# deflect-ca/banjax

Measured on AMD Instinct MI355X. Metric: log lines/sec matched+rate-limited (node) at 1k rules; HBM GB/s vs peak, higher is better.
Workload: dtype u8

## Files before the change

### banjax_amd/csrc/engine.hip

```cpp
#include <hip/hip_runtime.h>
#include <hipcub/hipcub.hpp>

#include <algorithm>
#include <array>
#include <atomic>
#include <cstdio>
#include <cstdlib>
#include <cstring>
#include <map>
#include <tuple>
#include <memory>
#include <mutex>
#include <stdexcept>
#include <string>
#include <unordered_map>
#include <thread>
#include <vector>

#include "../../include/banjax_gpu.h"
#include "bjx_common.h"
#include "engine_types.h"
#include "regex_compiler.h"
#include "bans.h"

// ... 379 lines not shown
  hid = host_lookup(B, p + host_off, host_len);
  exempt = B.any_allow && check_is_allowed(B, hid, p + ip_off, ip_len);
  L.ip_len[j] = ip_len;
  L.rest_off[j] = rest_off;
  L.host_id[j] = hid;
  {
    uint4 k16;
    uint64_t h;
    ip_key_hash(p + ip_off, ip_len, k16, h);
    if (ip_len > 15) L.ip_hash[j] = h;
    L.ip16[j] = k16;
  }
  if (!SLOW) {
    if (parse_float_fast(p, sp1, &f) != 0) {
      L.flags[j] = kLineSlowTs;
      unsigned long long k = atomicAdd(slow_count, 1ull);
      slow_list[k] = (uint32_t)j;
      return;
    }
  } else if (parse_float_fast(p, sp1, &f) != 0) {
    Decimal dec;
    if (go_parse_float(p, sp1, &f, &dec) != 0) { L.flags[j] = kLineError; return; }
  }
  const int64_t ts = ns_from_seconds(f);
  L.ts[j] = ts;
  if (go_sub(now_ns, ts) > 10000000000LL) fl = kLineOld;
  else if (exempt) fl = kLineExempt;
  L.flags[j] = fl;
  if (fl) return;

  const uint8_t *rest = p + rest_off;
  const uint32_t rest_len = n - rest_off;
  uint64_t word = 0;
  uint32_t pos = 0, wi = 0, nres = 0, nev = 0;
  uint32_t s_begin = 0, s_end = 0;
  if (hid >= 0) { s_begin = B.site_off[hid]; s_end = B.site_off[hid + 1]; }
  const uint32_t napp = (s_end - s_begin) + B.n_global;
  if (SLOW && napp > 128 && B.any_prefilter) {
    decide_wide(B, p, s, n, rest_off, hid, j, L, WL);
    return;
  }
  for (uint32_t k = 0; k < napp; ++k) {
    const uint32_t r = k < s_end - s_begin ? B.site_rules[s_begin + k] : B.global_rules[k - (s_end - s_begin)];
    if (B.any_wide && (B.rules[r].flags & kRuleNfaWide)) {
      const unsigned long long q = atomicAdd(WL.count, 1ull);
      if (q < WL.cap) { WL.line[q] = (uint32_t)j; WL.rule[q] = r; WL.pos[q] = pos; }
    } else if (rule_match(B, r, rest, rest_len)) {
      word |= 1ull << (pos & 63);
      ++nres;
      nev += is_skip(B, r, hid) ? 0u : 1u;
    }
    ++pos;
    if ((pos & 63) == 0) { L.mword(j, wi++) = word; word = 0; }
  }
  if (pos & 63) L.mword(j, wi) = word;
  L.counts[j] = ((uint64_t)nres << 32) | nev;
}

__global__ void k_no_line_pass(unsigned long long *slow_count, unsigned long long n) {
  if (threadIdx.x == 0) *slow_count = n;
}

template <bool SLOW>
__global__ __launch_bounds__(kBlock) void k_parse_match(Bind B, const uint8_t *__restrict__ buf,
                                                        const uint64_t *__restrict__ nl, uint64_t n_lines,
                                                        const uint32_t *__restrict__ list, int64_t now_ns, Lines L,
                                                        uint32_t *slow_list, unsigned long long *slow_count, WideList WL) {
  const uint64_t t = (uint64_t)blockIdx.x * blockDim.x + threadIdx.x;
  if (t >= n_lines) return;
  const uint64_t j = SLOW && list ? list[t] : t;
  const uint64_t s = j ? nl[j - 1] + 1 : 0;
  const uint32_t n = (uint32_t)(nl[j] - s);
  parse_and_match<SLOW>(B, buf + s, s, n, j, now_ns, L, slow_list, slow_count, WL);
}


constexpr uint32_t kWT = 4096;
constexpr uint32_t kHalo = 512;
constexpr uint32_t kLineCap = 128;
constexpr uint32_t kHitSlots = 4;
constexpr int kScanWaves = 16;
constexpr uint32_t kTileLds = kWT + kHalo + 16;
constexpr uint32_t kWaveJobs = 64;
constexpr uint32_t kCandList = 128;
constexpr uint32_t kBanChunks = 8;
constexpr uint64_t kBanChunkMin = 64ull << 20;
constexpr uint32_t kLongList = 64;
constexpr uint32_t kWaveLds = kTileLds + kLineCap * (2 + 2) + kCandList * 4 + kLineCap * 4 + kLongList * 8 + 16;
constexpr uint32_t kNone = 0xFFFFFFFFu;
constexpr uint32_t kScanLdsMax = 160 * 1024;
constexpr uint32_t kLinesImgMax = 16 * 1024;
constexpr uint32_t kLinesHostLdsMax = 6 * 1024;
constexpr uint32_t kLinesTabLdsMax = 10 * 1024;
constexpr uint32_t kLinesBlocksPerCu = 3;
constexpr uint32_t kSpanBytes = 12 * 1024;

__device__ __forceinline__ uint32_t space_mask16(const uint4 v) {
  const uint32_t wv[4] = {v.x, v.y, v.z, v.w};
  uint32_t m16 = 0;
#pragma unroll
  for (int k = 0; k < 4; ++k) {
    const uint32_t x = wv[k] ^ 0x20202020u;
    const uint32_t hb = ~(((x & 0x7F7F7F7Fu) + 0x7F7F7F7Fu) | x) & 0x80808080u;
    m16 |= (((hb >> 7) & 1u) | ((hb >> 14) & 2u) | ((hb >> 21) & 4u) | ((hb >> 28) & 8u)) << (4 * k);
  }
  return m16;
}

__device__ __forceinline__ bool digits4(uint32_t x) {
  return (x & 0xF0F0F0F0u) == 0x30303030u && (((x & 0x0F0F0F0Fu) + 0x06060606u) & 0xF0F0F0F0u) == 0u;
}
__device__ __forceinline__ uint32_t value4(uint32_t x) {
  x -= 0x30303030u;
  x = x * 10u + (x >> 8);
  return (x & 0xFFu) * 100u + ((x >> 16) & 0xFFu);
}
__device__ __forceinline__ int parse_ts_msec(const uint8_t *p, uint32_t n, double *out) {
  if (n != 14) return 1;
  const uint32_t w0 = ld4(p), w1 = ld4(p + 4), w2 = ld4(p + 8), w3 = ld4(p + 12);
  if (!digits4(w0) || !digits4(w1) || (w2 & 0x00FF0000u) != 0x002E0000u || !digits4((w2 & 0xFF00FFFFu) | 0x00300000u) ||
      !digits4((w3 & 0xFFFFu) | 0x30300000u))
    return 1;
  const uint32_t d8 = w2 & 0xFFu, d9 = (w2 >> 8) & 0xFFu, d11 = w2 >> 24, d12 = w3 & 0xFFu, d13 = (w3 >> 8) & 0xFFu;
  const uint64_t ip = (uint64_t)value4(w0) * 1000000ull + value4(w1) * 100u + (d8 - 48u) * 10u + (d9 - 48u);
  const uint64_t m = ip * 1000ull + (d11 - 48u) * 100u + (d12 - 48u) * 10u + (d13 - 48u);
  *out = (double)m / 1000.0;
  return 0;
}

__device__ __forceinline__ uint32_t find_spaces(const uint8_t *p, uint32_t n, uint32_t &sp0, uint32_t &sp1,
                                                uint32_t &sp2, uint32_t &sp3) {
  const uint32_t skip = (uint32_t)(reinterpret_cast<uintptr_t>(p) & 15);
  const uint4 *base = reinterpret_cast<const uint4 *>(p - skip);
  uint32_t ns = 0, c0 = 0;
  if (n + skip >= 64) {
    const uint4 v0 = base[0], v1 = base[1], v2 = base[2], v3 = base[3];
    uint64_t m = (uint64_t)space_mask16(v0) | ((uint64_t)space_mask16(v1) << 16) | ((uint64_t)space_mask16(v2) << 32) |
                 ((uint64_t)space_mask16(v3) << 48);
    m &= ~((1ull << skip) - 1ull);
#pragma unroll
    for (int k = 0; k < 4; ++k) {
      const uint32_t pos = (uint32_t)__ffsll((unsigned long long)m) - 1 - skip;
      const bool has = m != 0;
      m &= m - 1;
      if (k == 0) sp0 = has ? pos : sp0;
      if (k == 1) sp1 = has ? pos : sp1;
      if (k == 2) sp2 = has ? pos : sp2;
      if (k == 3) sp3 = has ? pos : sp3;
      ns += has ? 1u : 0u;
    }
    c0 = 4;
  }
  for (uint32_t c = c0; c * 16 < n + skip && ns < 4; ++c) {
    const uint4 v = base[c];
    uint32_t m16 = 0;
    const uint32_t wv[4] = {v.x, v.y, v.z, v.w};
#pragma unroll
    for (int k = 0; k < 4; ++k) {
      const uint32_t x = wv[k] ^ 0x20202020u;
      const uint32_t hb = ~(((x & 0x7F7F7F7Fu) + 0x7F7F7F7Fu) | x) & 0x80808080u;
      m16 |= (((hb >> 7) & 1u) | ((hb >> 14) & 2u) | ((hb >> 21) & 4u) | ((hb >> 28) & 8u)) << (4 * k);
    }
    const int32_t lo = (int32_t)skip - (int32_t)(c * 16), hi = lo + (int32_t)n;
    if (lo > 0) m16 &= ~((1u << lo) - 1u);
    if (hi < 16) m16 &= hi > 0 ? (1u << hi) - 1u : 0u;
    while (m16 && ns < 4) {
// ... 742 lines not shown
    const uint32_t lit = (uint32_t)(lits >> (16 * c)) & 0xFFFFu;
    if (lit != (a.y & 0xFFFFu) && lit != (a.y >> 16) && lit != (a.z & 0xFFFFu) && lit != (a.z >> 16)) continue;
    const uint32_t hp = (uint32_t)(lpos >> (16 * c)) & 0xFFFFu;
    if (hp == 0xFFFFu) {
      dfa_rule<EMIT>(B, T, r, pos, false, rest, rest_len, m0, m1, j, S);
      return;
    }
    const int32_t fs = side_c ? (int32_t)hp - (int32_t)host_len - (int32_t)la : (int32_t)hp;
    if (!tmpl_at(LT, a.w, rest, rest_len, host_rel, host_len, fs)) continue;
    if (eq) set_pos(m0, m1, pos);
    else dfa_rule<EMIT>(B, T, r, pos, false, rest, rest_len, m0, m1, j, S);
    return;
  }
}

template <bool EMIT>
__device__ __forceinline__ void decide_plan_lds(const Bind &B, const Tabs &T, const LdsTabs &LT, const uint8_t *rest,
                                                uint32_t rest_len, uint32_t host_rel, uint32_t host_len, int32_t hid,
                                                const HostRules &H, uint64_t lits, uint64_t lpos, uint32_t nlit, bool ovf,
                                                const OvfInfo &ov, uint64_t j, const Lines &L, const JobSink &S,
                                                LinesProf *P = nullptr) {
  const uint32_t nsite = H.s_end - H.s_begin;
  uint64_t m0 = H.a0, m1 = H.a1;
  if (P) { __builtin_amdgcn_s_waitcnt(0); P->mark(7); }
  if (hid >= 0) {
    const uint2 hi = LT.hinfo[hid];
    const uint32_t f = (uint32_t)__ffsll((unsigned long long)__ballot(1)) - 1;
    const uint32_t c0 = __builtin_amdgcn_readlane(hi.x, f);
    if (__ballot(hi.x != c0) == 0) {
      typedef const __attribute__((address_space(4))) uint32_t ConstU32;
      ConstU32 *cg = (ConstU32 *)(uintptr_t)(B.hl + B.lt_cls);
      const uint32_t cb = c0 & 0xFFFFu, ce = cb + (c0 >> 16);
      for (uint32_t i = cb; i < ce; ++i) {
        ConstU32 *q = cg + 8 * i;
        plan_rule_lds<EMIT>(B, T, LT, make_uint4(q[0], q[1], q[2], q[3]), make_uint4(q[4], q[5], q[6], q[7]), hi.y, rest, rest_len,
                            host_rel, host_len, lits, lpos, nlit, ovf, ov, m0, m1, j, S);
      }
    } else {
      const uint32_t cb = hi.x & 0xFFFFu, ce = cb + (hi.x >> 16);
      for (uint32_t i = cb; i < ce; ++i)
        plan_rule_lds<EMIT>(B, T, LT, LT.cls[2 * i], LT.cls[2 * i + 1], hi.y, rest, rest_len, host_rel, host_len, lits, lpos,
                            nlit, ovf, ov, m0, m1, j, S);
    }
  }
  if (P) { __builtin_amdgcn_s_waitcnt(0); P->mark(8); }
  for (uint32_t i = 0; i < B.n_plan_glob; ++i)
    plan_rule<EMIT>(B, T, B.plan_glob[2 * i], B.plan_glob[2 * i + 1], nsite, rest, rest_len, lits, lpos, nlit, ovf, ov, m0, m1,
                    j, S);
  if (P) { __builtin_amdgcn_s_waitcnt(0); P->mark(9); }
  L.mword(j, 0) = m0;
  if (B.mask_words > 1) L.mword(j, 1) = m1;
  const uint32_t nres = __popcll(m0) + __popcll(m1);
  const uint32_t nev = __popcll(m0 & ~H.k0) + __popcll(m1 & ~H.k1);
  L.counts[j] = ((uint64_t)nres << 32) | nev;
}

__device__ __forceinline__ void glds16(const void *g, void *lds) {
  __builtin_amdgcn_global_load_lds((const __attribute__((address_space(1))) void *)g,
                                   (__attribute__((address_space(3))) void *)lds, 16, 0, 0);
}

__device__ __forceinline__ void wave_sync() {
  __builtin_amdgcn_fence(__ATOMIC_RELEASE, "wavefront");
  __builtin_amdgcn_wave_barrier();
  __builtin_amdgcn_fence(__ATOMIC_ACQUIRE, "wavefront");
}

extern __shared__ __attribute__((aligned(16))) uint8_t s_dyn[];

__device__ __forceinline__ uint32_t wave_incl_sum(uint32_t v) {
  uint32_t x = v + (uint32_t)__builtin_amdgcn_update_dpp(0, (int)v, 0x111, 0xF, 0xF, false);
  x += (uint32_t)__builtin_amdgcn_update_dpp(0, (int)v, 0x112, 0xF, 0xF, false);
  x += (uint32_t)__builtin_amdgcn_update_dpp(0, (int)v, 0x113, 0xF, 0xF, false);
  x += (uint32_t)__builtin_amdgcn_update_dpp(0, (int)x, 0x114, 0xF, 0xE, false);
  x += (uint32_t)__builtin_amdgcn_update_dpp(0, (int)x, 0x118, 0xF, 0xC, false);
  x += (uint32_t)__builtin_amdgcn_update_dpp(0, (int)x, 0x142, 0xA, 0xF, false);
  x += (uint32_t)__builtin_amdgcn_update_dpp(0, (int)x, 0x143, 0xC, 0xF, false);
  return x;
}


template <bool IMG_LDS>
__global__ __launch_bounds__(kScanWaves * 64) __attribute__((amdgpu_waves_per_eu(4))) void k_scan(Bind B, ScanArgs A) {
  uint8_t *s_bits = s_dyn;
  uint8_t *s_img = s_dyn + kPairBytes;
  for (uint32_t i = threadIdx.x; i < kPairBytes / 16; i += blockDim.x)
    reinterpret_cast<uint4 *>(s_bits)[i] = reinterpret_cast<const uint4 *>(B.gram_pairs)[i];
  if (IMG_LDS)
    for (uint32_t i = threadIdx.x; i < B.scan_img_bytes / 16; i += blockDim.x)
      reinterpret_cast<uint4 *>(s_img)[i] = reinterpret_cast<const uint4 *>(B.scan_img)[i];
  __syncthreads();
  const Tabs TB = make_tabs(IMG_LDS ? s_img : B.scan_img, B.sil);
  const uint32_t *gt = TB.gt, *ge = TB.ge;

  const uint32_t lane = threadIdx.x & 63, wave = threadIdx.x >> 6;
  uint8_t *T = s_dyn + A.shared_bytes + wave * kWaveLds;
  uint16_t *ls = reinterpret_cast<uint16_t *>(T + kTileLds);
  uint16_t *le = ls + kLineCap;
  uint32_t *clist = reinterpret_cast<uint32_t *>(le + kLineCap);
  uint32_t *lcnt = clist + kCandList;
  uint64_t *lh = reinterpret_cast<uint64_t *>(lcnt + kLineCap);
  uint32_t *lh_n = reinterpret_cast<uint32_t *>(lh + kLongList);
  if (lane == 0) *lh_n = 0;
  const Lines &L = A.L;
  uint32_t n_probe = 0, n_hit = 0, n_gram = 0;

  const uint64_t nw = (uint64_t)gridDim.x * kScanWaves;
  uint64_t t = (uint64_t)blockIdx.x * kScanWaves + wave;
  uint4 q[4];
  uint2 qh;
  uint32_t qa;
  auto load_tile = [&](uint64_t tt) {
    const uint64_t ts = tt * kWT, base = ts + lane * 64u;
    if (base + 64 <= A.n) {
      const uint4 *src = reinterpret_cast<const uint4 *>(A.buf + base);
#pragma unroll
      for (int k = 0; k < 4; ++k) q[k] = src[k];
    } else {
      uint32_t w[16];
#pragma unroll
      for (int k = 0; k < 16; ++k) {
        uint32_t v = 0;
#pragma unroll
        for (int b = 0; b < 4; ++b) {
          const uint64_t pos = base + 4 * k + b;
          const uint32_t byte = A.buf[pos < A.n ? pos : A.n - 1];
          v |= (pos < A.n ? byte : 0u) << (8 * b);
        }
        w[k] = v;
      }
#pragma unroll
      for (int k = 0; k < 4; ++k) q[k] = make_uint4(w[4 * k], w[4 * k + 1], w[4 * k + 2], w[4 * k + 3]);
    }
    const uint64_t h = ts + kWT + lane * 8u;
    qh = make_uint2(0, 0);
    if (h + 8 <= A.n) qh = *reinterpret_cast<const uint2 *>(A.buf + h);
    else if (h < A.n) {
      uint32_t a = 0, b = 0;
#pragma unroll
      for (uint32_t k = 0; k < 8; ++k) {
        const uint64_t pos = h + k;
        const uint32_t byte = pos < A.n ? (uint32_t)A.buf[pos < A.n ? pos : A.n - 1] : 0u;
        if (k < 4) a |= byte << (8 * k); else b |= byte << (8 * (k - 4));
      }
      qh = make_uint2(a, b);
    }
    qa = 0x0A000000u;
    if (lane == 0) {
      if (tt) qa = *reinterpret_cast<const uint32_t *>(A.buf + ts - 4);
    } else if (lane <= 4 && (lane <= 2 || tt)) {
      qa = reinterpret_cast<const uint32_t *>(A.tile_base + tt - (lane <= 2 ? 0 : 1))[(lane - 1) & 1];
    }
  };
  auto flush_long = [&](uint64_t ts0, uint64_t tb, uint32_t nh) {
    wave_sync();
    const uint32_t nlh = min(*lh_n, kLongList);
    if (nlh == 0) return;
    const bool act = lane < nlh;
    const uint64_t e = act ? lh[lane] : 0;
    const uint32_t lsel = act ? (uint32_t)(e >> 13) & 0x1FFFu : kNone;
    const uint64_t gline = tb + nh + (uint64_t)lsel - 1u;
    uint32_t cc = 0;
    uint64_t pending = __ballot(act);
    while (pending) {
      const uint32_t l0 = (uint32_t)__ffsll((unsigned long long)pending) - 1;
      const uint32_t g = __builtin_amdgcn_readlane(lsel, l0);
      const uint64_t m = __ballot(act && lsel == g);
      uint32_t base = 0;
      if (lane == l0) base = atomicAdd(&L.cand_meta[gline].cnt, (uint32_t)__popcll(m));
      base = __builtin_amdgcn_readlane(base, l0);
      if (act && lsel == g) cc = base + (uint32_t)__popcll(m & ((1ull << lane) - 1ull));
      pending &= ~m;
    }
    if (act) {
      const uint32_t rel = (uint32_t)e & 0x1FFFu, lit = (uint32_t)(e >> 32) & 0xFFFFu;
      const uint64_t q0 = ts0 + rel - 256u;
      const uint64_t ver = ((e >> 26) & 1u) ? kCandVerified : 0ull;
      if (cc < (uint32_t)kCandSlots) {
        L.cand[gline * kCandSlots + cc] = (q0 << 24) | ver | lit;
      } else {
        const uint64_t bit = 1ull << (lit & 31);
        atomicOr(reinterpret_cast<unsigned long long *>(&L.cand_meta[gline].bits), ((e >> 27) & 1u) ? bit | (bit << 32) : bit);
        atomicMax(&L.cand_meta[gline].first_inv, ~(uint32_t)(q0 >> 3));
      }
    }
    wave_sync();
    if (lane == 0) *lh_n = 0;
    wave_sync();
  };

  const uint64_t n_iter = (A.n_tiles + nw - 1) / nw;
  if (t < A.n_tiles) load_tile(t);
  for (uint32_t r = 0; r < n_iter; ++r, t += nw) {
    if (t >= A.n_tiles) continue;
    const uint64_t ts0 = t * kWT;
    uint32_t w[16];
#pragma unroll
    for (int k = 0; k < 4; ++k) { w[4 * k] = q[k].x; w[4 * k + 1] = q[k].y; w[4 * k + 2] = q[k].z; w[4 * k + 3] = q[k].w; }
    const uint2 hv = qh;
    const uint32_t prevb = (uint32_t)__builtin_amdgcn_readlane(qa, 0) >> 24;
    const uint64_t tb = (uint64_t)(uint32_t)__builtin_amdgcn_readlane(qa, 1) | ((uint64_t)(uint32_t)__builtin_amdgcn_readlane(qa, 2) << 32);
    const uint64_t tbm = (uint64_t)(uint32_t)__builtin_amdgcn_readlane(qa, 3) | ((uint64_t)(uint32_t)__builtin_amdgcn_readlane(qa, 4) << 32);
    const uint32_t prev_cnt = t ? (uint32_t)(tb - tbm) : 0u;
    if (t + nw < A.n_tiles) load_tile(t + nw);
    uint4 *dst = reinterpret_cast<uint4 *>(T + lane * 64u);
#pragma unroll
    for (int k = 0; k < 4; ++k) dst[k] = make_uint4(w[4 * k], w[4 * k + 1], w[4 * k + 2], w[4 * k + 3]);
    *reinterpret_cast<uint2 *>(T + kWT + lane * 8u) = hv;
    if (lane < 4) reinterpret_cast<uint32_t *>(T + kWT + kHalo)[lane] = 0;

    uint64_t nlm;
    {
      uint32_t nb[8];
#pragma unroll
      for (int i = 0; i < 8; ++i) {
        const uint32_t d = __builtin_amdgcn_udot4(nl_mask_word(w[2 * i]), 0x08040201u, 0u, false);
        nb[i] = __builtin_amdgcn_udot4(nl_mask_word(w[2 * i + 1]), 0x80402010u, d, false) >> 7;
      }
      const uint32_t lo32 = nb[0] | (nb[1] << 8) | (nb[2] << 16) | (nb[3] << 24);
      const uint32_t hi32 = nb[4] | (nb[5] << 8) | (nb[6] << 16) | (nb[7] << 24);
      nlm = ((uint64_t)hi32 << 32) | lo32;
    }
    const uint32_t cnt = __popcll(nlm);
    uint32_t pre = wave_incl_sum(cnt);
    const uint32_t tot = __builtin_amdgcn_readlane(pre, 63);
    pre -= cnt;
    const bool head = prevb == '\n';
    const uint32_t nh = head ? 0u : 1u;
    const bool last_nl = (__shfl((uint32_t)(nlm >> 63), 63) & 1u) != 0;
    const uint32_t n_st = (head ? 1u : 0u) + tot - (last_nl ? 1u : 0u);
    const uint64_t any_nl = __ballot(cnt != 0);
    uint32_t p0 = kNone;
    if (any_nl) {
      const uint32_t fl = (uint32_t)__ffsll((unsigned long long)any_nl) - 1;
      const uint64_t fm = __shfl(nlm, fl);
      p0 = fl * 64u + (uint32_t)__ffsll((unsigned long long)fm) - 1;
    }
    uint32_t hmask;
    {
      const uint32_t a = nl_mask_word(hv.x), b = nl_mask_word(hv.y);
      hmask = ((a >> 7) & 1u) | ((a >> 14) & 2u) | ((a >> 21) & 4u) | ((a >> 28) & 8u) |
              (((b >> 7) & 1u) | ((b >> 14) & 2u) | ((b >> 21) & 4u) | ((b >> 28) & 8u)) << 4;
    }
    if (ts0 + kWT + lane * 8u >= A.n) hmask = 0;
    const uint64_t any_h = __ballot(hmask != 0);
    uint32_t hfirst = kNone;
    if (any_h) {
      const uint32_t fl = (uint32_t)__ffsll((unsigned long long)any_h) - 1;
      hfirst = kWT + fl * 8u + (uint32_t)__ffs(__shfl(hmask, fl)) - 1;
    }
    {
      uint64_t x = nlm;
      uint32_t rr = pre;
      while (x) {
        const uint32_t b = (uint32_t)__ffsll((unsigned long long)x) - 1;
        x &= x - 1;
        const uint32_t p = lane * 64u + b;
        if (tb + rr < A.n_lines) A.nl[tb + rr] = ts0 + p;
        const int32_t lk = (int32_t)rr - (int32_t)nh;
        if (lk >= 0 && lk < (int32_t)kLineCap) le[lk] = (uint16_t)p;
        if (p + 1 < kWT && lk + 1 < (int32_t)kLineCap) ls[lk + 1] = (uint16_t)(p + 1);
        ++rr;
      }
    }
    if (lane == 0 && head) ls[0] = 0;
    const bool last_in_halo = n_st && !last_nl && hfirst != kNone;
    const bool last_long = n_st && !last_nl && hfirst == kNone;
    if (lane == 0 && last_in_halo && n_st - 1 < kLineCap) le[n_st - 1] = (uint16_t)hfirst;
    wave_sync();
    if (!B.any_prefilter || (A.debug_skip & 1)) continue;
    const uint64_t win_end = A.n - ts0 < (uint64_t)(kWT + kHalo) ? A.n - ts0 : (uint64_t)(kWT + kHalo);
    const bool open_long = !head && (p0 == kNone || p0 >= kHalo || prev_cnt == 0);
    const uint32_t hend = last_in_halo ? hfirst : kWT;

    {
      const uint32_t nxt = *reinterpret_cast<const uint32_t *>(T + lane * 64u + 64u);
      uint32_t hlo = 0, hhi = 0;
#pragma unroll
      for (int k0 = 0; k0 < 64; k0 += 16) {
        uint2 ent[8];
#pragma unroll
        for (int i = 0; i < 8; ++i) {
          const int k = k0 + 2 * i;
          const uint32_t lo = w[k >> 2], hi = (k >> 2) < 15 ? w[(k >> 2) + 1] : nxt;
          const uint32_t g1 = __builtin_amdgcn_alignbyte(hi, lo, (uint32_t)(k & 3) + 1u);
          ent[i] = *reinterpret_cast<const uint2 *>(s_bits + gram_pair_byte_off(g1));
        }
#pragma unroll
        for (int i = 0; i < 8; ++i) {
          const int k = k0 + 2 * i;
          const uint32_t lo = w[k >> 2], hi = (k >> 2) < 15 ? w[(k >> 2) + 1] : nxt;
          const uint32_t g0 = (k & 3) ? __builtin_amdgcn_alignbyte(hi, lo, (uint32_t)(k & 3)) : lo;
          const uint32_t g1 = __builtin_amdgcn_alignbyte(hi, lo, (uint32_t)(k & 3) + 1u);
          const uint32_t two = __builtin_amdgcn_ubfe(ent[i].x, g0, 1) | (__builtin_amdgcn_ubfe(ent[i].y, g1 >> 24, 1) << 1);
          if (k < 32) hlo |= two << k; else hhi |= two << (k - 32);
        }
      }
      uint64_t hits = ((uint64_t)hhi << 32) | hlo;
      if (ts0 + lane * 64u + 64u > A.n) hits &= (ts0 + lane * 64u >= A.n) ? 0ull : ((1ull << (A.n - ts0 - lane * 64u)) - 1ull);
      uint32_t hh = 0;
      if (lane * 8u + kWT < hend) {
        const uint32_t hw[3] = {hv.x, hv.y, *reinterpret_cast<const uint32_t *>(T + kWT + lane * 8u + 8u)};
        uint2 ent[4];
#pragma unroll
        for (int i = 0; i < 4; ++i) {
          const int k = 2 * i;
          const uint32_t g1 = __builtin_amdgcn_alignbyte(hw[(k >> 2) + 1], hw[k >> 2], (uint32_t)(k & 3) + 1u);
          ent[i] = *reinterpret_cast<const uint2 *>(s_bits + gram_pair_byte_off(g1));
        }
#pragma unroll
        for (int i = 0; i < 4; ++i) {
          const int k = 2 * i;
          const uint32_t lo = hw[k >> 2], hi = hw[(k >> 2) + 1];
          const uint32_t g0 = (k & 3) ? __builtin_amdgcn_alignbyte(hi, lo, (uint32_t)(k & 3)) : lo;
          const uint32_t g1 = __builtin_amdgcn_alignbyte(hi, lo, (uint32_t)(k & 3) + 1u);
          hh |= (__builtin_amdgcn_ubfe(ent[i].x, g0, 1) | (__builtin_amdgcn_ubfe(ent[i].y, g1 >> 24, 1) << 1)) << k;
        }
        const uint32_t nv = hend - (kWT + lane * 8u);
        if (nv < 8) hh &= (1u << nv) - 1u;
      }
      n_probe += __popcll(hits) + __popc(hh);
      if (A.debug_skip & 2) { hits = 0; hh = 0; }
      for (uint32_t i = lane; i < kLineCap; i += 64) lcnt[i] = 0;
      uint64_t rem = hits;
      uint32_t remh = hh;
      for (;;) {
        const uint32_t cn = __popcll(rem) + __popc(remh);
        uint32_t off = wave_incl_sum(cn);
        const uint32_t total = __builtin_amdgcn_readlane(off, 63);
        if (total == 0) break;
        off -= cn;
        while ((rem | remh) && off < kCandList) {
          uint32_t pos;
          int32_t lk;
          if (rem) {
            const uint32_t k = (uint32_t)__ffsll((unsigned long long)rem) - 1;
            rem &= rem - 1;
            pos = lane * 64u + k;
            lk = (int32_t)(pre + (uint32_t)__popcll(nlm & ((1ull << k) - 1ull))) - (int32_t)nh;
          } else {
            const uint32_t k = (uint32_t)__ffs(remh) - 1;
            remh &= remh - 1;
            pos = kWT + lane * 8u + k;
            lk = (int32_t)n_st - 1;
          }
          clist[off++] = pos | ((uint32_t)(lk + 1) << 16);
        }
        wave_sync();
        const uint32_t nc = total < kCandList ? total : kCandList;
        for (uint32_t c = lane; c < nc; c += 64) {
          const uint32_t en0 = clist[c];
          const uint32_t s = en0 & 0xFFFF;
          const int32_t lk = (int32_t)(en0 >> 16) - 1;
          const uint32_t g = ld4(T + s);
          if ((g & 0xFF) == '\n' || (A.debug_skip & 8)) continue;
          uint32_t slot = gram_slot(g, B.gt2_cap);
          uint32_t ol;
          for (;;) {
            ol = gt[2 * slot + 1];
            if ((ol & 0xFFFF) == 0 || gt[2 * slot] == g) break;
            slot = (slot + 1) & (B.gt2_cap - 1);
          }
          if ((ol & 0xFFFF) == 0) continue;
          ++n_gram;
          if (A.debug_skip & 4) continue;
          if (lk < 0 && !open_long) continue;
          const uint64_t gline = tb + nh + (uint64_t)(int64_t)lk;
          if (gline >= A.n_lines) continue;
          const bool in_window = lk >= 0 && lk < (int32_t)kLineCap && !(lk == (int32_t)n_st - 1 && last_long);
          for (uint32_t ei = 0; ei < (ol & 0xFFFF); ++ei) {
            const uint32_t en = ge[(ol >> 16) + ei];
            const uint32_t lit = en >> 8, goff = en & 0xFF;
            const int64_t q0 = (int64_t)(ts0 + s) - (int64_t)goff;
            if (q0 < 0) continue;
            const int32_t s0 = (int32_t)s - (int32_t)goff;
            if (in_window) {
              if (s0 < (int32_t)ls[lk] || (uint32_t)s0 + lit_len_of(TB, lit) > le[lk]) continue;
              if (!literal_at16(TB, lit, T + s0)) continue;
              const uint32_t cc = atomicAdd(&lcnt[lk], 1u);
              if (B.cfirst) atomicMin(reinterpret_cast<unsigned long long *>(&L.cand_first[gline * kCandFirstLits + lit]),
                                      (unsigned long long)q0);
              if (cc < (uint32_t)kCandSlots) {
                L.cand[gline * kCandSlots + cc] = ((uint64_t)q0 << 24) | kCandVerified | lit;
              } else {
                const bool far = s0 - (int32_t)ls[lk] >= (int32_t)kCertainGap;
                const uint64_t bit = 1ull << (lit & 31);
                atomicOr(reinterpret_cast<unsigned long long *>(&L.cand_meta[gline].bits), far ? bit | (bit << 32) : bit);
                atomicMax(&L.cand_meta[gline].first_inv, ~(uint32_t)((uint64_t)q0 >> 3));
              }
            } else {
              bool ver = false;
              if (s0 >= 0 && !B.lit_nl && (uint64_t)s0 + lit_len_of(TB, lit) <= win_end) {
                if (!literal_at16(TB, lit, T + s0)) continue;
                ver = true;
              }
              if (B.cfirst) atomicMin(reinterpret_cast<unsigned long long *>(&L.cand_first[gline * kCandFirstLits + lit]),
                                      (unsigned long long)q0);
              const bool far = lk < 0 ? s0 >= (int32_t)kCertainGap
                                      : lk < (int32_t)kLineCap && s0 - (int32_t)ls[lk] >= (int32_t)kCertainGap;
              const uint32_t at = atomicAdd(lh_n, 1u);
// ... 4605 lines not shown
      if (sn) HIP_OK(hipMemcpy(sample.data(), bytes, sn, hipMemcpyDeviceToHost));
      sp = sample.data();
    }
    bind_ruleset(e, rs, sp, sn);
  }
  const Bind &B = e->bind;
  hipStream_t st = e->stream;
  memset(out, 0, sizeof *out);
  e->trips.clear();
  e->trips_c.clear();
  e->results.clear();
  e->line_flags.clear();
  if (n == 0) return false;

  const uint8_t *buf = bytes;
  if (!(flags & BJX_INPUT_DEVICE) || (reinterpret_cast<uintptr_t>(bytes) & 15)) {
    e->staging.ensure(n + 16);
    HIP_OK(hipMemcpyAsync(e->staging.p, bytes, n, (flags & BJX_INPUT_DEVICE) ? hipMemcpyDeviceToDevice : hipMemcpyHostToDevice, st));
    buf = e->staging.p;
  }
  HIP_OK(hipEventRecord(e->ev0, st));
  for (auto &r : e->phase_rec) r = false;
  mark(e, 0);

  const uint64_t n_tiles = (n + kWT - 1) / kWT;
  e->tile_counts.ensure(n_tiles);
  e->tile_base.ensure(n_tiles + 1);
  uint64_t n_lines = 0;
  Lines L;
  hipLaunchKernelGGL(k_nl_count_wt, dim3((unsigned)((n_tiles + 3) / 4)), dim3(kBlock), 0, st, buf, (uint64_t)n, n_tiles,
                     e->tile_counts.p);
  HIP_OK(hipGetLastError());
  {
    uint32_t *in = e->tile_counts.p;
    uint64_t *o = e->tile_base.p;
    cub_call(e, [&](void *tmp, size_t &bytes) { return hipcub::DeviceScan::ExclusiveSum(tmp, bytes, in, o, (int)n_tiles, st); });
  }
  {
    uint64_t last_base = 0;
    uint32_t last_cnt = 0;
    pin_get(e, &last_base, e->tile_base.p + (n_tiles - 1), 8);
    pin_get(e, &last_cnt, e->tile_counts.p + (n_tiles - 1), 4);
    pin_sync(e);
    n_lines = last_base + last_cnt;
  }
  out->n_lines = n_lines;
  if (n_lines == 0) return false;
  const uint64_t cap = n_lines;

  e->nl.ensure(cap);
  e->l_ts.ensure(cap); e->l_iph.ensure(cap); e->l_counts.ensure(cap + 1); e->l_offs.ensure(cap + 1);
  e->l_masks.ensure(cap * B.mask_words);
  e->l_iplen.ensure(cap);
  e->l_roff.ensure(cap); e->l_hid.ensure(cap); e->l_flags.ensure(cap); e->slow_list.ensure(cap);
  e->l_ccnt.ensure(cap); e->l_ip16.ensure(cap);
  e->l_cand.ensure(B.any_prefilter ? cap * kCandSlots : 1);
  e->scalars.ensure(16);
  L.ts = e->l_ts.p; L.ip_hash = e->l_iph.p; L.ip_len = e->l_iplen.p;
  L.rest_off = e->l_roff.p; L.host_id = e->l_hid.p; L.flags = e->l_flags.p;
  L.counts = e->l_counts.p; L.masks = e->l_masks.p; L.mstride = cap;
  L.cand_meta = e->l_ccnt.p; L.cand = e->l_cand.p; L.ip16 = e->l_ip16.p;
  L.cand_first = nullptr;
  if (B.cfirst) {
    e->l_cfirst.ensure(cap * kCandFirstLits);
    L.cand_first = e->l_cfirst.p;
    HIP_OK(hipMemsetAsync(e->l_cfirst.p, 0xFF, cap * kCandFirstLits * 8, st));
  }
  e->jline.ensure(std::max<uint64_t>(e->jline.n, cap + (1u << 20)));
  e->jkey.ensure(e->jline.n); e->jidx.ensure(e->jline.n); e->jrec.ensure(e->jline.n);
  HIP_OK(hipMemsetAsync(e->scalars.p, 0, 16 * sizeof(unsigned long long), st));
  if (B.any_prefilter) HIP_OK(hipMemsetAsync(e->l_ccnt.p, 0, cap * sizeof(CandMeta), st));
  mark(e, 1);

  {
    int n_cu_scan = 0;
    HIP_OK(hipDeviceGetAttribute(&n_cu_scan, hipDeviceAttributeMultiprocessorCount, e->device));
    const unsigned scan_grid = (unsigned)std::min<uint64_t>((n_tiles + kScanWaves - 1) / kScanWaves, (uint64_t)std::max(1, n_cu_scan));
    ScanArgs A;
    A.buf = buf; A.n = n; A.n_tiles = n_tiles; A.n_lines = cap; A.tile_base = e->tile_base.p; A.nl = e->nl.p;
    A.L = L; A.stats = e->scalars.p + 8;
    A.debug_skip = getenv("BJX_DEBUG_SKIP") ? (uint32_t)atoi(getenv("BJX_DEBUG_SKIP")) : 0u;
    const uint32_t fixed = kPairBytes + kScanWaves * kWaveLds;
    const bool img_lds = fixed + B.scan_img_bytes <= kScanLdsMax;
    A.shared_bytes = kPairBytes + (img_lds ? B.scan_img_bytes : 0);
    const uint32_t lds = A.shared_bytes + kScanWaves * kWaveLds;
    using ScanFn = void (*)(Bind, ScanArgs);
    const ScanFn kfn = img_lds ? k_scan<true> : k_scan<false>;
    if (lds != e->scan_lds[img_lds]) {
      HIP_OK(hipFuncSetAttribute(reinterpret_cast<const void *>(kfn), hipFuncAttributeMaxDynamicSharedMemorySize, (int)lds));
      e->scan_lds[img_lds] = lds;
    }
    HIP_OK(hipEventRecord(e->evm0, st));
    hipLaunchKernelGGL(kfn, dim3(scan_grid), dim3(kScanWaves * 64), lds, st, B, A);
    HIP_OK(hipGetLastError());
    HIP_OK(hipEventRecord(e->evm1, st));
  }
  uint64_t last_nl = 0;
  mark(e, 2);

  unsigned long long sc4[5] = {0, 0, 0, 0, 0};
  unsigned long long n_jobs = 0;
  const bool all_wide = B.n_global > 128 && !(getenv("BJX_LINES") && atoi(getenv("BJX_LINES")) == 1);
  int n_cu = 0;
  HIP_OK(hipDeviceGetAttribute(&n_cu, hipDeviceAttributeMultiprocessorCount, e->device));
  if (!e->lines_attr) {
    for (const void *f : {reinterpret_cast<const void *>(&k_lines<true>), reinterpret_cast<const void *>(&k_lines<false>),
#ifdef BJX_PROF
                          reinterpret_cast<const void *>(&k_lines<true, true>),
                          reinterpret_cast<const void *>(&k_lines<false, true>),
                          reinterpret_cast<const void *>(&k_lines<true, true, true>),
                          reinterpret_cast<const void *>(&k_lines<false, true, true>),
#endif
                          reinterpret_cast<const void *>(&k_lines<true, false, true>),
                          reinterpret_cast<const void *>(&k_lines<false, false, true>)})
      HIP_OK(hipFuncSetAttribute(f, hipFuncAttributeMaxDynamicSharedMemorySize, (int)kScanLdsMax));
    e->lines_attr = true;
  }
  auto resident_grid = [&](const void *fn, uint32_t lds, uint64_t work) {
    int per_cu = 0;
    HIP_OK(hipOccupancyMaxActiveBlocksPerMultiprocessor(&per_cu, fn, kBlock, lds));
    const uint64_t resident = (uint64_t)std::max(1, per_cu) * (uint64_t)std::max(1, n_cu);
    return (unsigned)std::max<uint64_t>(1, std::min<uint64_t>((work + kBlock - 1) / kBlock, resident));
  };
  for (int attempt = 0;; ++attempt) {
    LinesArgs A;
    A.buf = buf; A.n = n; A.nl = e->nl.p; A.n_lines = n_lines; A.L = L; A.now_ns = now_ns;
    A.dbg = getenv("BJX_DEBUG_LINES") ? (uint32_t)atoi(getenv("BJX_DEBUG_LINES")) : 0u;
    A.dbg2 = getenv("BJX_DEBUG_L2") ? (uint32_t)atoi(getenv("BJX_DEBUG_L2")) : 0u;
    A.slow_list = e->slow_list.p; A.slow_count = e->scalars.p;
    A.jline = e->jline.p; A.jkey = e->jkey.p; A.jidx = e->jidx.p; A.jrec = e->jrec.p; A.job_count = e->scalars.p + 11;
    A.job_cap = std::min(std::min(e->jline.n, e->jkey.n), std::min(e->jidx.n, e->jrec.n));
    A.job_real = e->scalars.p + 14;
    A.null_key = 2 * B.n_rules;
    A.span_bytes = getenv("BJX_SPAN_BYTES") ? (uint32_t)atoi(getenv("BJX_SPAN_BYTES")) & ~15u : kSpanBytes;
    A.list = nullptr; A.n_list = 0; A.prof = nullptr;
    HIP_OK(hipEventRecord(e->evk[0], st));
    static const int lines_env = getenv("BJX_LINES") ? atoi(getenv("BJX_LINES")) : 2;
    const bool use_l2 = B.l2_bytes && lines_env != 1 && !getenv("BJX_PROF_LINES") && !A.dbg;
    e->last_line_kernel = all_wide ? 3u : use_l2 ? 2u : 1u;
    if (all_wide) {
      hipLaunchKernelGGL(k_no_line_pass, dim3(1), dim3(64), 0, st, e->scalars.p, (unsigned long long)n_lines);
      HIP_OK(hipGetLastError());
    } else if (use_l2) {
      const uint32_t lds = B.l2_bytes + (kL2Block / 64) * kL2WaveLds;
      const void *fn = B.l2_w == 2 ? reinterpret_cast<const void *>(&k_lines2<2>) : reinterpret_cast<const void *>(&k_lines2<1>);
      if (lds != e->lines2_lds || B.l2_w != e->lines2_w) {
        HIP_OK(hipFuncSetAttribute(fn, hipFuncAttributeMaxDynamicSharedMemorySize, (int)lds));
        e->lines2_lds = lds;
        e->lines2_w = B.l2_w;
      }
      int per_cu = 0;
      HIP_OK(hipOccupancyMaxActiveBlocksPerMultiprocessor(&per_cu, fn, kL2Block, lds));
      const uint64_t resident = (uint64_t)std::max(1, per_cu) * (uint64_t)std::max(1, n_cu);
      const unsigned grid = (unsigned)std::max<uint64_t>(1, std::min<uint64_t>((n_lines + kL2Block - 1) / kL2Block, resident));
      static const bool dbg_img = getenv("BJX_DEBUG_IMG") != nullptr;
      if (dbg_img) fprintf(stderr, "[bjx] k_lines2: %u B LDS per block (tables %u), %d blocks per CU, grid %u\n", lds, B.l2_bytes, per_cu, grid);
#ifdef BJX_PROF_L2
      e->chk.ensure(16);
      HIP_OK(hipMemsetAsync(e->chk.p, 0, 128, st));
      A.prof = e->chk.p;
#endif
      if (B.l2_w == 2) hipLaunchKernelGGL(k_lines2<2>, dim3(grid), dim3(kL2Block), lds, st, B, A);
      else hipLaunchKernelGGL(k_lines2<1>, dim3(grid), dim3(kL2Block), lds, st, B, A);
      HIP_OK(hipGetLastError());
#ifdef BJX_PROF_L2
      {
        unsigned long long c[8];
// ... 1127 lines not shown
```

### banjax_amd/csrc/engine_types.h

```cpp
#pragma once
#include <stdint.h>

namespace bjx {

struct DevRule {
  uint32_t trans_off;
  uint32_t ae_off;
  uint32_t na_off;
  uint16_t n_na;
  uint16_t ncls;
  uint16_t start;
  uint16_t flags;
  uint32_t name_id;
  int32_t decision;
  uint32_t lits_off;
  uint16_t lits_len;
  uint8_t mode;
  uint8_t equiv;
  uint32_t anc_off;
  uint16_t anc_len;
  uint8_t anc_equiv;
  uint8_t lead;
  uint32_t n_states;
  int64_t interval_ns;
  int64_t hits;
  uint32_t nfa_off;
  uint32_t nfa_words;
  uint16_t skip_len;
  uint16_t skip_state;
  uint16_t lead_dist;
};

constexpr uint32_t kJiNfa = 1, kJiEquiv = 2, kJiBigLit = 16;

constexpr uint32_t kPairEntries = 2048;
constexpr uint32_t kPairBytes = kPairEntries * 8;
constexpr uint32_t kGramMul = 0x2C1B3Bu;
__host__ __device__ inline uint32_t gram_mix(uint32_t x) {
#ifdef __HIP_DEVICE_COMPILE__
  return __umul24(x, kGramMul);
#else
  return (x & 0xFFFFFFu) * kGramMul;
#endif
}
__host__ __device__ inline uint32_t gram_pair_index(uint32_t key) { return (gram_mix(key) >> 13) & (kPairEntries - 1); }
__host__ __device__ inline uint32_t gram_pair_byte_off(uint32_t key) { return (gram_mix(key) >> 10) & ((kPairEntries - 1) << 3); }
__host__ __device__ inline uint32_t gram_slot(uint32_t g, uint32_t cap) { return ((g * 0x9E3779B1u) >> 14) & (cap - 1); }
constexpr int kCandSlots = 4;
constexpr uint64_t kCandVerified = 1u << 23;

struct Subnet {
  uint8_t net[16];
  uint8_t mask[16];
  uint32_t netlen;
  uint32_t _pad;
};

struct ImgLayout {
  uint32_t gt, ge, ht, hrec, hid, hbytes, lrec, lbytes, lcim, lchk;
};

struct HostSlot {
  uint32_t tag;
  int32_t id;
  uint32_t len;
  uint32_t off;
  uint8_t inl[48];
};

struct Bind {
  const DevRule *rules;
  const uint4 *jinfo;
  const uint16_t *trans;
  const uint8_t *accept_end;
  const uint32_t *accel;
  const uint8_t *ascii_cls;
  const uint32_t *nonascii;
  const uint8_t *lits;
  const uint32_t *global_rules;
  const uint32_t *site_off;
  const uint32_t *site_rules;
  const uint64_t *hd_hash;
  const uint32_t *hd_id;
  const uint32_t *hd_off;
  const uint32_t *hd_len;
  const uint8_t *hd_bytes;
  const HostSlot *hslot;
  const int32_t *host_scope;
  const uint64_t *skip_keys;
  const uint32_t *sc_addr_off;
  const uint64_t *sc_addr;
  const uint32_t *sc_sub_off;
  const Subnet *sc_sub;
  const uint32_t *sc_str_off;
  const uint64_t *sc_str_hash;
  const uint32_t *sc_str_boff;
  const uint32_t *sc_str_len;
  const uint8_t *sc_str_bytes;
  uint32_t n_rules;
  uint32_t n_global;
  uint32_t n_hosts;
  uint32_t n_hd;
  uint32_t n_skip;
  uint32_t n_scopes;
  uint32_t any_allow;
  uint32_t mask_words;
  const uint2 *gram_pairs;
  const uint32_t *rule_lits;
  uint32_t n_lits;
  uint32_t any_anchored;
  uint32_t any_prefilter;
  uint32_t lits_small;
  uint32_t lit_nl;
  uint32_t cfirst;
  ImgLayout il;
  const uint8_t *img;
  uint32_t img_bytes;
  const uint8_t *scan_img;
  uint32_t scan_img_bytes;
  ImgLayout sil;
  uint32_t gt2_cap, gt2_nent;
  uint32_t ht_cap;
  uint32_t max_app;
// ... 151 lines not shown
```

Before: 2.390 billion.

## Restructure scan loop prefetch, fast-path full tiles, move gram pairs to static LDS

Reworks the k_scan tile loop into a software pipeline that loads the next tile before processing the current one, and adds a fast path for full tiles that skips per-byte bounds checks. The newline index stores become packed uint2 writes, and bit extraction switches to alignbit shift-in accumulation. The gram pair table moves into static shared memory, and the wave index is made uniform via readfirstlane. An inline-asm v_mul_u32_u24 is used in gram_mix. The aim is to cut ALU work and hide load latency in the hot scan kernel, but it raises register pressure and carries correctness risk in the reordered hit-bit packing.

```diff
diff --git a/banjax_amd/csrc/engine.hip b/banjax_amd/csrc/engine.hip
--- a/banjax_amd/csrc/engine.hip
+++ b/banjax_amd/csrc/engine.hip
@@ -485,6 +485,7 @@
 constexpr int kScanWaves = 16;
 constexpr uint32_t kTileLds = kWT + kHalo + 16;
 constexpr uint32_t kWaveJobs = 64;
+constexpr int kScanGroup = 8;
 constexpr uint32_t kCandList = 128;
 constexpr uint32_t kBanChunks = 8;
 constexpr uint64_t kBanChunkMin = 64ull << 20;
@@ -1393,10 +1394,10 @@
 
 template <bool IMG_LDS>
 __global__ __launch_bounds__(kScanWaves * 64) __attribute__((amdgpu_waves_per_eu(4))) void k_scan(Bind B, ScanArgs A) {
-  uint8_t *s_bits = s_dyn;
-  uint8_t *s_img = s_dyn + kPairBytes;
+  __shared__ __attribute__((aligned(16))) uint2 s_pairs[kPairEntries];
+  uint8_t *s_img = s_dyn;
   for (uint32_t i = threadIdx.x; i < kPairBytes / 16; i += blockDim.x)
-    reinterpret_cast<uint4 *>(s_bits)[i] = reinterpret_cast<const uint4 *>(B.gram_pairs)[i];
+    reinterpret_cast<uint4 *>(s_pairs)[i] = reinterpret_cast<const uint4 *>(B.gram_pairs)[i];
   if (IMG_LDS)
     for (uint32_t i = threadIdx.x; i < B.scan_img_bytes / 16; i += blockDim.x)
       reinterpret_cast<uint4 *>(s_img)[i] = reinterpret_cast<const uint4 *>(B.scan_img)[i];
@@ -1404,7 +1405,7 @@
   const Tabs TB = make_tabs(IMG_LDS ? s_img : B.scan_img, B.sil);
   const uint32_t *gt = TB.gt, *ge = TB.ge;
 
-  const uint32_t lane = threadIdx.x & 63, wave = threadIdx.x >> 6;
+  const uint32_t lane = threadIdx.x & 63, wave = __builtin_amdgcn_readfirstlane(threadIdx.x >> 6);
   uint8_t *T = s_dyn + A.shared_bytes + wave * kWaveLds;
   uint16_t *ls = reinterpret_cast<uint16_t *>(T + kTileLds);
   uint16_t *le = ls + kLineCap;
@@ -1417,12 +1418,11 @@
   uint32_t n_probe = 0, n_hit = 0, n_gram = 0;
 
   const uint64_t nw = (uint64_t)gridDim.x * kScanWaves;
-  uint64_t t = (uint64_t)blockIdx.x * kScanWaves + wave;
-  uint4 q[4];
-  uint2 qh;
-  uint32_t qa;
-  auto load_tile = [&](uint64_t tt) {
-    const uint64_t ts = tt * kWT, base = ts + lane * 64u;
+  const uint64_t t_first = (uint64_t)blockIdx.x * kScanWaves + wave;
+  uint4 q[4] = {make_uint4(0, 0, 0, 0), make_uint4(0, 0, 0, 0), make_uint4(0, 0, 0, 0), make_uint4(0, 0, 0, 0)};
+  uint2 qh = make_uint2(0, 0);
+  uint32_t qa = 0;
+  auto load_tile_edge = [&](uint64_t ts, uint64_t base) __attribute__((always_inline)) {
     if (base + 64 <= A.n) {
       const uint4 *src = reinterpret_cast<const uint4 *>(A.buf + base);
 #pragma unroll
@@ -1455,6 +1455,18 @@
         if (k < 4) a |= byte << (8 * k); else b |= byte << (8 * (k - 4));
       }
       qh = make_uint2(a, b);
+    }
+  };
+  auto load_tile = [&](uint64_t tt) __attribute__((always_inline)) {
+    const uint64_t ts = tt * kWT, base = ts + lane * 64u;
+    const bool full = ts + kWT + kHalo <= A.n;
+    if (__builtin_expect(full, 1)) {
+      const uint4 *src = reinterpret_cast<const uint4 *>(A.buf + base);
+#pragma unroll
+      for (int k = 0; k < 4; ++k) q[k] = src[k];
+      qh = *reinterpret_cast<const uint2 *>(A.buf + ts + kWT + lane * 8u);
+    } else {
+      load_tile_edge(ts, base);
     }
     qa = 0x0A000000u;
     if (lane == 0) {
@@ -1500,20 +1512,27 @@
     wave_sync();
   };
 
-  const uint64_t n_iter = (A.n_tiles + nw - 1) / nw;
-  if (t < A.n_tiles) load_tile(t);
-  for (uint32_t r = 0; r < n_iter; ++r, t += nw) {
-    if (t >= A.n_tiles) continue;
+  bool have = false;
+  uint64_t tc = 0;
+  for (uint64_t tl = t_first;; tl += nw) {
+    const bool more = tl < A.n_tiles;
+    if (!have && !more) break;
+    const uint4 q0 = q[0], q1 = q[1], q2 = q[2], q3 = q[3];
+    const uint2 hv = qh;
+    const uint32_t qa0 = qa;
+    if (more) load_tile(tl);
+    const bool cur = have;
+    const uint64_t t = tc;
+    have = more;
+    tc = tl;
+    if (!cur) continue;
     const uint64_t ts0 = t * kWT;
-    uint32_t w[16];
-#pragma unroll
-    for (int k = 0; k < 4; ++k) { w[4 * k] = q[k].x; w[4 * k + 1] = q[k].y; w[4 * k + 2] = q[k].z; w[4 * k + 3] = q[k].w; }
-    const uint2 hv = qh;
-    const uint32_t prevb = (uint32_t)__builtin_amdgcn_readlane(qa, 0) >> 24;
-    const uint64_t tb = (uint64_t)(uint32_t)__builtin_amdgcn_readlane(qa, 1) | ((uint64_t)(uint32_t)__builtin_amdgcn_readlane(qa, 2) << 32);
-    const uint64_t tbm = (uint64_t)(uint32_t)__builtin_amdgcn_readlane(qa, 3) | ((uint64_t)(uint32_t)__builtin_amdgcn_readlane(qa, 4) << 32);
+    const bool edge = t == 0 || t + 1 >= A.n_tiles || ts0 + kWT + kHalo > A.n;
+    const uint32_t w[16] = {q0.x, q0.y, q0.z, q0.w, q1.x, q1.y, q1.z, q1.w, q2.x, q2.y, q2.z, q2.w, q3.x, q3.y, q3.z, q3.w};
+    const uint32_t prevb = (uint32_t)__builtin_amdgcn_readlane(qa0, 0) >> 24;
+    const uint64_t tb = (uint64_t)(uint32_t)__builtin_amdgcn_readlane(qa0, 1) | ((uint64_t)(uint32_t)__builtin_amdgcn_readlane(qa0, 2) << 32);
+    const uint64_t tbm = (uint64_t)(uint32_t)__builtin_amdgcn_readlane(qa0, 3) | ((uint64_t)(uint32_t)__builtin_amdgcn_readlane(qa0, 4) << 32);
     const uint32_t prev_cnt = t ? (uint32_t)(tb - tbm) : 0u;
-    if (t + nw < A.n_tiles) load_tile(t + nw);
     uint4 *dst = reinterpret_cast<uint4 *>(T + lane * 64u);
 #pragma unroll
     for (int k = 0; k < 4; ++k) dst[k] = make_uint4(w[4 * k], w[4 * k + 1], w[4 * k + 2], w[4 * k + 3]);
@@ -1553,7 +1572,7 @@
       hmask = ((a >> 7) & 1u) | ((a >> 14) & 2u) | ((a >> 21) & 4u) | ((a >> 28) & 8u) |
               (((b >> 7) & 1u) | ((b >> 14) & 2u) | ((b >> 21) & 4u) | ((b >> 28) & 8u)) << 4;
     }
-    if (ts0 + kWT + lane * 8u >= A.n) hmask = 0;
+    if (edge && ts0 + kWT + lane * 8u >= A.n) hmask = 0;
     const uint64_t any_h = __ballot(hmask != 0);
     uint32_t hfirst = kNone;
     if (any_h) {
@@ -1563,11 +1582,15 @@
     {
       uint64_t x = nlm;
       uint32_t rr = pre;
+      uint2 *nl_t = reinterpret_cast<uint2 *>(A.nl + tb);
+      const uint64_t room64 = tb < A.n_lines ? A.n_lines - tb : 0;
+      const uint32_t room = room64 < (uint64_t)kWT ? (uint32_t)room64 : kWT;
+      const uint32_t ts_lo = (uint32_t)ts0, ts_hi = (uint32_t)(ts0 >> 32);
       while (x) {
         const uint32_t b = (uint32_t)__ffsll((unsigned long long)x) - 1;
         x &= x - 1;
         const uint32_t p = lane * 64u + b;
-        if (tb + rr < A.n_lines) A.nl[tb + rr] = ts0 + p;
+        if (rr < room) nl_t[rr] = make_uint2(ts_lo | p, ts_hi);
         const int32_t lk = (int32_t)rr - (int32_t)nh;
         if (lk >= 0 && lk < (int32_t)kLineCap) le[lk] = (uint16_t)p;
         if (p + 1 < kWT && lk + 1 < (int32_t)kLineCap) ls[lk + 1] = (uint16_t)(p + 1);
@@ -1586,29 +1609,36 @@
 
     {
       const uint32_t nxt = *reinterpret_cast<const uint32_t *>(T + lane * 64u + 64u);
+      auto gram_at = [](const uint32_t *wd, int k) -> uint32_t {
+        return (k & 3) ? __builtin_amdgcn_alignbyte(wd[(k >> 2) + 1], wd[k >> 2], (uint32_t)(k & 3)) : wd[k >> 2];
+      };
+      auto push_bit = [](uint32_t acc, uint32_t word, uint32_t byte) -> uint32_t {
+        return __builtin_amdgcn_alignbit(word >> (byte & 31u), acc, 1u);
+      };
+      uint32_t wx[17];
+#pragma unroll
+      for (int k = 0; k < 16; ++k) wx[k] = w[k];
+      wx[16] = nxt;
       uint32_t hlo = 0, hhi = 0;
 #pragma unroll
-      for (int k0 = 0; k0 < 64; k0 += 16) {
-        uint2 ent[8];
+      for (int k0 = 0; k0 < 64; k0 += 2 * kScanGroup) {
+        uint2 ent[kScanGroup];
 #pragma unroll
-        for (int i = 0; i < 8; ++i) {
+        for (int i = 0; i < kScanGroup; ++i) {
           const int k = k0 + 2 * i;
-          const uint32_t lo = w[k >> 2], hi = (k >> 2) < 15 ? w[(k >> 2) + 1] : nxt;
-          const uint32_t g1 = __builtin_amdgcn_alignbyte(hi, lo, (uint32_t)(k & 3) + 1u);
-          ent[i] = *reinterpret_cast<const uint2 *>(s_bits + gram_pair_byte_off(g1));
+          const uint32_t g1 = __builtin_amdgcn_alignbyte(wx[(k >> 2) + 1], wx[k >> 2], (uint32_t)(k & 3) + 1u);
+          ent[i] = s_pairs[gram_pair_byte_off(g1) >> 3];
         }
 #pragma unroll
-        for (int i = 0; i < 8; ++i) {
+        for (int i = 0; i < kScanGroup; ++i) {
           const int k = k0 + 2 * i;
-          const uint32_t lo = w[k >> 2], hi = (k >> 2) < 15 ? w[(k >> 2) + 1] : nxt;
-          const uint32_t g0 = (k & 3) ? __builtin_amdgcn_alignbyte(hi, lo, (uint32_t)(k & 3)) : lo;
-          const uint32_t g1 = __builtin_amdgcn_alignbyte(hi, lo, (uint32_t)(k & 3) + 1u);
-          const uint32_t two = __builtin_amdgcn_ubfe(ent[i].x, g0, 1) | (__builtin_amdgcn_ubfe(ent[i].y, g1 >> 24, 1) << 1);
-          if (k < 32) hlo |= two << k; else hhi |= two << (k - 32);
+          const uint32_t b4 = k + 4 <= 64 ? gram_at(wx, k + 4) : nxt >> 16;
+          if (k < 32) hlo = push_bit(push_bit(hlo, ent[i].x, gram_at(wx, k)), ent[i].y, b4);
+          else hhi = push_bit(push_bit(hhi, ent[i].x, gram_at(wx, k)), ent[i].y, b4);
         }
       }
       uint64_t hits = ((uint64_t)hhi << 32) | hlo;
-      if (ts0 + lane * 64u + 64u > A.n) hits &= (ts0 + lane * 64u >= A.n) ? 0ull : ((1ull << (A.n - ts0 - lane * 64u)) - 1ull);
+      if (edge && ts0 + lane * 64u + 64u > A.n) hits &= (ts0 + lane * 64u >= A.n) ? 0ull : ((1ull << (A.n - ts0 - lane * 64u)) - 1ull);
       uint32_t hh = 0;
       if (lane * 8u + kWT < hend) {
         const uint32_t hw[3] = {hv.x, hv.y, *reinterpret_cast<const uint32_t *>(T + kWT + lane * 8u + 8u)};
@@ -1617,16 +1647,15 @@
         for (int i = 0; i < 4; ++i) {
           const int k = 2 * i;
           const uint32_t g1 = __builtin_amdgcn_alignbyte(hw[(k >> 2) + 1], hw[k >> 2], (uint32_t)(k & 3) + 1u);
-          ent[i] = *reinterpret_cast<const uint2 *>(s_bits + gram_pair_byte_off(g1));
+          ent[i] = s_pairs[gram_pair_byte_off(g1) >> 3];
         }
 #pragma unroll
         for (int i = 0; i < 4; ++i) {
           const int k = 2 * i;
-          const uint32_t lo = hw[k >> 2], hi = hw[(k >> 2) + 1];
-          const uint32_t g0 = (k & 3) ? __builtin_amdgcn_alignbyte(hi, lo, (uint32_t)(k & 3)) : lo;
-          const uint32_t g1 = __builtin_amdgcn_alignbyte(hi, lo, (uint32_t)(k & 3) + 1u);
-          hh |= (__builtin_amdgcn_ubfe(ent[i].x, g0, 1) | (__builtin_amdgcn_ubfe(ent[i].y, g1 >> 24, 1) << 1)) << k;
+          const uint32_t b4 = k + 4 <= 8 ? gram_at(hw, k + 4) : hw[2] >> 16;
+          hh = push_bit(push_bit(hh, ent[i].x, gram_at(hw, k)), ent[i].y, b4);
         }
+        hh >>= 24;
         const uint32_t nv = hend - (kWT + lane * 8u);
         if (nv < 8) hh &= (1u << nv) - 1u;
       }
@@ -6398,7 +6427,7 @@
     A.debug_skip = getenv("BJX_DEBUG_SKIP") ? (uint32_t)atoi(getenv("BJX_DEBUG_SKIP")) : 0u;
     const uint32_t fixed = kPairBytes + kScanWaves * kWaveLds;
     const bool img_lds = fixed + B.scan_img_bytes <= kScanLdsMax;
-    A.shared_bytes = kPairBytes + (img_lds ? B.scan_img_bytes : 0);
+    A.shared_bytes = img_lds ? B.scan_img_bytes : 0;
     const uint32_t lds = A.shared_bytes + kScanWaves * kWaveLds;
     using ScanFn = void (*)(Bind, ScanArgs);
     const ScanFn kfn = img_lds ? k_scan<true> : k_scan<false>;
diff --git a/banjax_amd/csrc/engine_types.h b/banjax_amd/csrc/engine_types.h
--- a/banjax_amd/csrc/engine_types.h
+++ b/banjax_amd/csrc/engine_types.h
@@ -38,7 +38,9 @@
 constexpr uint32_t kGramMul = 0x2C1B3Bu;
 __host__ __device__ inline uint32_t gram_mix(uint32_t x) {
 #ifdef __HIP_DEVICE_COMPILE__
-  return __umul24(x, kGramMul);
+  uint32_t m;
+  asm("v_mul_u32_u24 %0, %1, %2" : "=v"(m) : "s"(kGramMul), "v"(x));
+  return m;
 #else
   return (x & 0xFFFFFFu) * kGramMul;
 #endif
```

Result: faster. 2.437 billion (median of 6 runs) (+2.0%).
